# NVIDIA/nccl

Measured on AMD Instinct MI355X. Metric: all-reduce bus GB/s (device-resident), 256 MiB fp32, 1/2/4/8 MI355X, higher is better.
Workload: dtype f32; 1 GPU; ncclAllReduce sum fp32, 256 MiB, world_size=1 (the metric's size at N=1); collective=ncclAllReduce, op=sum, bytes_per_rank=268435456, count=67108864, n_ranks=1, out_of_place=True

## Files before the change

### nccl_amd/csrc/enqueue.cc

```cpp
#include <errno.h>
#include <stdio.h>
#include <stdlib.h>
#include <string.h>

#include <algorithm>
#include <cmath>

#include "core.h"

namespace ncclamd {

int typeSize(ncclDataType_t t) {
  switch (t) {
    case ncclInt8: case ncclUint8: case ncclFloat8e4m3: case ncclFloat8e5m2: return 1;
    case ncclFloat16: case ncclBfloat16: return 2;
    case ncclInt32: case ncclUint32: case ncclFloat32: return 4;
    case ncclInt64: case ncclUint64: case ncclFloat64: return 8;
    default: return -1;
  }
}

static uint16_t hostF32ToHalf(float f);
static uint16_t hostF32ToBf16(float f);
static uint8_t hostF32ToFp8(float f, bool e5m2);
// ... 258 lines not shown
      if (!strcmp(a, "*")) lo = 1, hi = NCCL_AMD_MAX_RANKS;
      else if (end != a && *end == '\0' && nr >= 1 && nr <= NCCL_AMD_MAX_RANKS) lo = hi = (int)nr;
      if (lo && okB && okC && okD) {
        for (int n = lo; n <= hi; n++) {
          if (vb >= 0) t->tableLL[n] = vb;
          if (vc >= 0) t->tableLL128[n] = vc;
          if (vd >= 0) t->tableOneShot[n] = vd;
        }
        rows++;
        continue;
      }
    }
    WARN("NCCL_AMD_SIZE_TABLE=%s:%d: expected 'nranks|* ll ll128 oneshot' (bytes, K/M/G, '-' = built-in); line ignored",
         path, lineNo);
    good = false;
  }
  fclose(f);
  INFO("NCCL_AMD_SIZE_TABLE=%s: %d rows applied", path, rows);
  return good;
}

int linkChannelBudget(int n) {
  if (n < 3) return 0;
  const double bLinkGBps = 76.8, wgGBps = 23.0, headroom = 2.0;
  const double need = (2.5 * n - 1.0) * bLinkGBps / wgGBps * headroom;
  int c = 32;
  while (c < need && c < NCCL_AMD_MAX_CHANNELS) c *= 2;
  return c;
}

int coResidentChannelCap(int minCUs, int ranksPerGpu) {
  if (minCUs < 1) minCUs = 256;
  if (ranksPerGpu < 1) ranksPerGpu = 1;
  const int cap = ranksPerGpu == 1 ? 2 * minCUs : minCUs / ranksPerGpu;
  return cap < 1 ? 1 : cap;
}

void resolveLinkChannels(CommTuning* t, int nranks, bool userMaxCTAs) {
  const int64_t env = paramInt("NCCL_AMD_LINK_CHANNELS", -1);
  t->linkChannels = env >= 0 ? (int)env : userMaxCTAs ? 0 : linkChannelBudget(nranks);
}

void resolveFence(CommTuning* t, bool oneDevice) {
  if (t->p2pFence < 0 && oneDevice) t->protoFlags |= 8;
}

static bool isHostMemory(const void* p) {
// ... 763 lines not shown
```

### nccl_amd/csrc/kernels.h

```cpp
#pragma once
#include <hip/hip_runtime.h>

#include <algorithm>
#include <type_traits>

#include "core.h"
#include "numerics.h"

namespace ncclamd {

typedef unsigned int u32x4 __attribute__((ext_vector_type(4)));
constexpr int kThreads = 512;
#define kCoResident __attribute__((amdgpu_waves_per_eu(4)))

extern bool gKernelLog;
void kernelLogNote(const void* fn, unsigned grid, unsigned block);
#define NCCL_AMD_LAUNCH(K, G, B, SH, ST, ...)                                                  \
  do {                                                                                          \
    if (::ncclamd::gKernelLog) ::ncclamd::kernelLogNote((const void*)(K), (G).x, (B).x);      \
    hipLaunchKernelGGL(K, G, B, SH, ST, __VA_ARGS__);                                           \
  } while (0)


__device__ __forceinline__ uint64_t clockTicks() { return __builtin_amdgcn_s_memrealtime(); }

__device__ __forceinline__ void storeRemote(void* p, u32x4 v) {
  asm volatile("global_store_dwordx4 %0, %1, off sc0 sc1\n\ts_nop 1" ::"v"(p), "v"(v) : "memory");
}
__device__ __forceinline__ void drainStores() { asm volatile("s_waitcnt vmcnt(0)" ::: "memory"); }

#ifndef NCCL_AMD_BUFFER_STORES
#define NCCL_AMD_BUFFER_STORES 1
#endif
constexpr int kSysWriteThrough = 1 | 16;
__device__ __forceinline__ __amdgpu_buffer_rsrc_t remoteRsrc(const void* base) {
  const uint64_t b = (uint64_t)base;
  const uint32_t lo = __builtin_amdgcn_readfirstlane((uint32_t)b);
  const uint32_t hi = __builtin_amdgcn_readfirstlane((uint32_t)(b >> 32));
  return __builtin_amdgcn_make_buffer_rsrc((void*)(((uint64_t)hi << 32) | lo), 0, -1, 0x00020000);
}
__device__ __forceinline__ void storeRemoteAt(__amdgpu_buffer_rsrc_t r, uint32_t byteOff, u32x4 v) {
  __builtin_amdgcn_raw_buffer_store_b128(v, r, byteOff, 0, kSysWriteThrough);
}

#ifndef NCCL_AMD_LOCAL_WT
#define NCCL_AMD_LOCAL_WT 0
#endif
struct LocalStore {
  __amdgpu_buffer_rsrc_t r;
  u32x4* d;
  __device__ __forceinline__ LocalStore(void* dst, uint64_t base) : d((u32x4*)dst + base) {
    if (NCCL_AMD_LOCAL_WT) r = remoteRsrc(d);
  }
  __device__ __forceinline__ void put(uint32_t k, u32x4 v) {
    if (NCCL_AMD_LOCAL_WT) __builtin_amdgcn_raw_buffer_store_b128(v, r, k * 16u, 0, kSysWriteThrough);
    else __builtin_nontemporal_store(v, d + k);
  }
};

template <typename T>
__device__ __forceinline__ void storeRemoteElt(T* p, T v) {
  if constexpr (sizeof(T) == 1) {
    uint32_t x = 0;
    __builtin_memcpy(&x, &v, 1);
    asm volatile("global_store_byte %0, %1, off sc0 sc1\n\ts_nop 1" ::"v"(p), "v"(x) : "memory");
  } else if constexpr (sizeof(T) == 2) {
    uint32_t x = 0;
    __builtin_memcpy(&x, &v, 2);
    asm volatile("global_store_short %0, %1, off sc0 sc1\n\ts_nop 1" ::"v"(p), "v"(x) : "memory");
  } else if constexpr (sizeof(T) == 4) {
    uint32_t x;
    __builtin_memcpy(&x, &v, 4);
    asm volatile("global_store_dword %0, %1, off sc0 sc1\n\ts_nop 1" ::"v"(p), "v"(x) : "memory");
  } else {
    uint64_t x;
    __builtin_memcpy(&x, &v, 8);
    asm volatile("global_store_dwordx2 %0, %1, off sc0 sc1\n\ts_nop 1" ::"v"(p), "v"(x) : "memory");
  }
}
// ... 101 lines not shown
#ifndef NCCL_AMD_COPY_UNROLL
#define NCCL_AMD_COPY_UNROLL 8
#endif
constexpr int kCopyUnroll = NCCL_AMD_COPY_UNROLL;
#ifndef NCCL_AMD_FOLD_UNROLL
#define NCCL_AMD_FOLD_UNROLL 4
#endif
constexpr int kFoldUnroll = NCCL_AMD_FOLD_UNROLL;
#ifndef NCCL_AMD_FOLD_UNROLL_SWAR
#define NCCL_AMD_FOLD_UNROLL_SWAR 2
#endif
#ifndef NCCL_AMD_FOLD_UNROLL_1B
#define NCCL_AMD_FOLD_UNROLL_1B 2
#endif
constexpr int kFoldUnrollSwar = NCCL_AMD_FOLD_UNROLL_SWAR;
constexpr int kFoldUnroll1B = NCCL_AMD_FOLD_UNROLL_1B;
#ifndef NCCL_AMD_FOLD_REPACK
#define NCCL_AMD_FOLD_REPACK 1
#endif
#ifndef NCCL_AMD_FOLD_PREFETCH
#define NCCL_AMD_FOLD_PREFETCH 1
#endif

template <typename T, bool REMOTE>
__device__ __forceinline__ void copyRange(void* dst, const void* src, uint64_t nbytes, bool aligned) {
  if (aligned) {
    uint64_t npk = nbytes >> 4;
    const u32x4* s = (const u32x4*)src;
    u32x4* d = (u32x4*)dst;
    constexpr int U = kCopyUnroll;
    uint64_t i = threadIdx.x;
    for (; i + (U - 1) * kThreads < npk; i += U * kThreads) {
      u32x4 v[U];
#pragma unroll
      for (int u = 0; u < U; u++) v[u] = __builtin_nontemporal_load(s + i + u * kThreads);
      LocalStore ls(dst, i - threadIdx.x);
      __amdgpu_buffer_rsrc_t rd;
      if (REMOTE && NCCL_AMD_BUFFER_STORES) rd = remoteRsrc(d + (i - threadIdx.x));
#pragma unroll
      for (int u = 0; u < U; u++) {
        if (REMOTE && NCCL_AMD_BUFFER_STORES) storeRemoteAt(rd, (uint32_t)((threadIdx.x + u * kThreads) * 16), v[u]);
        else if (REMOTE) storeRemote(d + i + u * kThreads, v[u]);
        else ls.put(threadIdx.x + u * kThreads, v[u]);
      }
    }
    for (; i < npk; i += kThreads) {
      u32x4 v = __builtin_nontemporal_load(s + i);
      if (REMOTE && NCCL_AMD_BUFFER_STORES) storeRemoteAt(remoteRsrc(d + (i - threadIdx.x)), threadIdx.x * 16u, v);
      else if (REMOTE) storeRemote(d + i, v);
      else __builtin_nontemporal_store(v, d + i);
    }
    uint64_t done = npk << 4;
    uint64_t tail = (nbytes - done) / sizeof(T);
    if (threadIdx.x < tail) {
      const T* st = (const T*)((const char*)src + done);
      T* dt = (T*)((char*)dst + done);
      if (REMOTE) storeRemoteElt(dt + threadIdx.x, st[threadIdx.x]);
      else dt[threadIdx.x] = st[threadIdx.x];
    }
  } else {
    uint64_t n = nbytes / sizeof(T);
    const T* s = (const T*)src;
    T* d = (T*)dst;
    for (uint64_t i = threadIdx.x; i < n; i += kThreads) {
      if (REMOTE) storeRemoteElt(d + i, s[i]);
      else d[i] = s[i];
    }
  }
}

template <typename T>
__device__ __forceinline__ void copyRangeMulti(char* dstLocal, char* const* dstPush, int nPush, const void* src,
                                               uint64_t nbytes, bool aligned) {
  if (nPush == 1 && !dstLocal) return copyRange<T, true>(dstPush[0], src, nbytes, aligned);
  if (nPush == 0) return dstLocal ? copyRange<T, false>(dstLocal, src, nbytes, aligned) : void();
  if (aligned) {
    const uint64_t npk = nbytes >> 4;
    const u32x4* s = (const u32x4*)src;
    constexpr int U = kCopyUnroll;
    uint64_t i = threadIdx.x;
    for (; i + (U - 1) * kThreads < npk; i += U * kThreads) {
      u32x4 v[U];
#pragma unroll
      for (int u = 0; u < U; u++) v[u] = __builtin_nontemporal_load(s + i + u * kThreads);
      if (dstLocal) {
        LocalStore ls(dstLocal, i - threadIdx.x);
#pragma unroll
        for (int u = 0; u < U; u++) ls.put(threadIdx.x + u * kThreads, v[u]);
      }
      for (int p = 0; p < nPush; p++) {
        u32x4* d = (u32x4*)dstPush[p];
        if (NCCL_AMD_BUFFER_STORES) {
          const __amdgpu_buffer_rsrc_t rd = remoteRsrc(d + (i - threadIdx.x));
#pragma unroll
          for (int u = 0; u < U; u++) storeRemoteAt(rd, (uint32_t)((threadIdx.x + u * kThreads) * 16), v[u]);
        } else {
#pragma unroll
          for (int u = 0; u < U; u++) storeRemote(d + i + u * kThreads, v[u]);
        }
      }
    }
    for (; i < npk; i += kThreads) {
      const u32x4 v = __builtin_nontemporal_load(s + i);
      if (dstLocal) __builtin_nontemporal_store(v, (u32x4*)dstLocal + i);
      for (int p = 0; p < nPush; p++) {
        u32x4* d = (u32x4*)dstPush[p];
        if (NCCL_AMD_BUFFER_STORES) storeRemoteAt(remoteRsrc(d + (i - threadIdx.x)), threadIdx.x * 16u, v);
        else storeRemote(d + i, v);
      }
    }
    const uint64_t done = npk << 4;
    const uint64_t tail = (nbytes - done) / sizeof(T);
    if (threadIdx.x < tail) {
      const T x = ((const T*)((const char*)src + done))[threadIdx.x];
      if (dstLocal) ((T*)(dstLocal + done))[threadIdx.x] = x;
      for (int p = 0; p < nPush; p++) storeRemoteElt((T*)(dstPush[p] + done) + threadIdx.x, x);
    }
  } else {
    const uint64_t n = nbytes / sizeof(T);
    const T* s = (const T*)src;
    for (uint64_t i = threadIdx.x; i < n; i += kThreads) {
      const T x = s[i];
      if (dstLocal) ((T*)dstLocal)[i] = x;
      for (int p = 0; p < nPush; p++) storeRemoteElt((T*)dstPush[p] + i, x);
    }
  }
}

template <typename T>
union PackU {
  u32x4 v;
  T e[16 / sizeof(T)];
};

template <typename T, int OP>
__device__ __forceinline__ u32x4 fp8PackF32(const Red<T, OP>& fn, int n, const char* const* src, uint64_t i) {
  constexpr bool E5 = IsFp8<T>::e5m2;
  u32x4 cur = __builtin_nontemporal_load((const u32x4*)src[0] + i), nxt = cur;
  float acc[16];
  for (int k = 0; k < n; k++) {
    if (k + 1 < n) nxt = __builtin_nontemporal_load((const u32x4*)src[k + 1] + i);
    float x[16];
#pragma unroll
    for (int w = 0; w < 4; w++) fp8Decode4<E5>(cur[w], x + 4 * w);
    if constexpr (OP == DEV_PREMULSUM) {
#pragma unroll
      for (int e = 0; e < 16; e += 2) {
        x[e] = opaqueF(x[e] * fn.s);
        x[e + 1] = opaqueF(x[e + 1] * fn.s);
        fp8RoundF<E5>(x[e], x[e + 1]);
      }
    }
    if (k == 0) {
#pragma unroll
      for (int e = 0; e < 16; e++) acc[e] = x[e];
    } else {
#pragma unroll
      for (int e = 0; e < 16; e += 2) {
        float r0, r1;
        if (OP == DEV_PROD) {
          r0 = opaqueF(x[e] * acc[e]);
          r1 = opaqueF(x[e + 1] * acc[e + 1]);
        } else if (OP == DEV_MINMAX) {
          r0 = fn.isMin ? minOrdered(x[e], acc[e]) : maxOrdered(x[e], acc[e]);
// ... 9 lines not shown
    }
    cur = nxt;
  }
  u32x4 out;
#pragma unroll
  for (int w = 0; w < 4; w++) out[w] = fp8Encode4<E5>(acc + 4 * w);
  return out;
}

#ifndef NCCL_AMD_FP8_H2
#define NCCL_AMD_FP8_H2 1
#endif
template <typename T, int OP>
__device__ __forceinline__ void foldFp8Packs(const Red<T, OP>& fn, int n, const char* const* src, uint64_t nelem,
                                             char* dstLocal, char* const* dstPush, int nPush) {
  constexpr bool E5 = IsFp8<T>::e5m2;
  const uint64_t npk = nelem / 16;
  const _Float16 sh = (_Float16)fn.s;
  const fp8h2 s2 = {sh, sh};
  const uint32_t scalarSpecial = (OP == DEV_PREMULSUM && !(__builtin_fabsf(fn.s) <= 65504.0f)) ? 1u : 0u;
  for (uint64_t i = threadIdx.x; i < npk; i += kThreads) {
    u32x4 out;
    if (NCCL_AMD_FP8_H2) {
      u32x4 cur = __builtin_nontemporal_load((const u32x4*)src[0] + i), nxt = cur;
      fp8h2 acc[8];
      uint32_t special = scalarSpecial;
      for (int k = 0; k < n; k++) {
        if (k + 1 < n) nxt = __builtin_nontemporal_load((const u32x4*)src[k + 1] + i);
        special |= fp8Special<E5>(cur[0]) | fp8Special<E5>(cur[1]) | fp8Special<E5>(cur[2]) | fp8Special<E5>(cur[3]);
        fp8h2 x[8];
#pragma unroll
        for (int w = 0; w < 4; w++) {
          x[2 * w] = fp8DecodeH2<E5>(cur[w], false);
          x[2 * w + 1] = fp8DecodeH2<E5>(cur[w], true);
        }
        if constexpr (OP == DEV_PREMULSUM) {
#pragma unroll
          for (int j = 0; j < 8; j++) x[j] = fp8RoundH2<E5>(x[j] * s2);
        }
        if (k == 0) {
#pragma unroll
          for (int j = 0; j < 8; j++) acc[j] = x[j];
        } else {
#pragma unroll
          for (int j = 0; j < 8; j++) {
            if (OP == DEV_MINMAX)
              acc[j] = fn.isMin ? __builtin_elementwise_minimum(x[j], acc[j]) : __builtin_elementwise_maximum(x[j], acc[j]);
            else if (OP == DEV_PROD)
              acc[j] = fp8RoundH2<E5>(x[j] * acc[j]);
            else
              acc[j] = fp8RoundH2<E5>(x[j] + acc[j]);
          }
        }
        cur = nxt;
      }
#pragma unroll
      for (int w = 0; w < 4; w++) out[w] = fp8EncodeH2x2<E5>(acc[2 * w], acc[2 * w + 1]);
      if (__builtin_expect(special != 0, 0)) out = fp8PackF32<T, OP>(fn, n, src, i);
    } else {
      out = fp8PackF32<T, OP>(fn, n, src, i);
    }
    if (dstLocal) __builtin_nontemporal_store(out, (u32x4*)dstLocal + i);
    for (int p = 0; p < nPush; p++) storeRemoteAt(remoteRsrc((u32x4*)dstPush[p] + (i - threadIdx.x)), threadIdx.x * 16u, out);
  }
  const uint64_t t = npk * 16 + threadIdx.x;
  if (t < nelem) {
    T a = fn.pre(((const T*)src[0])[t]);
    for (int k = 1; k < n; k++) a = fn.red(fn.pre(((const T*)src[k])[t]), a);
    a = fn.post(a);
    if (dstLocal) ((T*)dstLocal)[t] = a;
    for (int p = 0; p < nPush; p++) storeRemoteElt((T*)dstPush[p] + t, a);
  }
}

template <typename T, int OP, int UMAX = 64>
__device__ __forceinline__ void foldRange(const Red<T, OP>& fn, int n, const char* const* src, uint64_t nelem,
                                          char* dstLocal, char* const* dstPush, int nPush, bool aligned) {
  constexpr int EPP = 16 / sizeof(T);
  constexpr bool kSwarDiv = std::is_same<T, uint8_t>::value && OP == DEV_SUMPOSTDIV;
  constexpr bool kSwar = std::is_same<T, uint8_t>::value && (Swar8<OP>::ok || kSwarDiv);
  constexpr int kSwarOp = kSwarDiv ? DEV_SUM : OP;
  constexpr int U0 = sizeof(T) > 1 ? kFoldUnroll : kSwar ? kFoldUnrollSwar : kFoldUnroll1B;
  constexpr int U = U0 < UMAX ? U0 : UMAX;
  uint32_t swarMask = 0, divMagic = 0;
  if constexpr (kSwar && !kSwarDiv) swarMask = (uint32_t)(uint8_t)fn.arg * 0x01010101u;
  if constexpr (kSwarDiv) divMagic = swarDivMagic(fn.divisor);
  if constexpr (IsFp8<T>::value && NCCL_AMD_HW_FP8) {
    if (aligned) {
      foldFp8Packs<T, OP>(fn, n, src, nelem, dstLocal, dstPush, nPush);
      return;
    }
  }
  if (aligned) {
    const uint64_t npk = nelem / EPP;
    const uint64_t step = (uint64_t)U * kThreads;
    constexpr bool kPrefetch = NCCL_AMD_FOLD_PREFETCH && sizeof(T) > 1;
    PackU<T> acc[U], cur[U], nxt[U];
    if constexpr (kPrefetch) {
#pragma unroll
      for (int u = 0; u < U; u++) {
        uint64_t i = threadIdx.x + (uint64_t)u * kThreads;
        if (i < npk) cur[u].v = __builtin_nontemporal_load((const u32x4*)src[0] + i);
      }
    }
    for (uint64_t base = threadIdx.x; base < npk; base += step) {
      if constexpr (!kPrefetch) {
#pragma unroll
        for (int u = 0; u < U; u++) {
          uint64_t i = base + (uint64_t)u * kThreads;
          if (i < npk) cur[u].v = __builtin_nontemporal_load((const u32x4*)src[0] + i);
        }
      }
      for (int k = 0; k < n; k++) {
        const bool last = k + 1 == n;
        if (!last || (kPrefetch && base + step < npk)) {
          const u32x4* s = (const u32x4*)src[last ? 0 : k + 1];
          const uint64_t b = last ? base + step : base;
#pragma unroll
          for (int u = 0; u < U; u++) {
            uint64_t i = b + (uint64_t)u * kThreads;
            if (i < npk) nxt[u].v = __builtin_nontemporal_load(s + i);
          }
        }
#pragma unroll
        for (int u = 0; u < U; u++) {
          if constexpr (kSwar) {
#pragma unroll
            for (int w = 0; w < 4; w++) acc[u].v[w] = k == 0 ? cur[u].v[w] : Swar8<kSwarOp>::red(cur[u].v[w], acc[u].v[w], swarMask);
          } else {
#pragma unroll
            for (int e = 0; e < EPP; e++) {
              T x = fn.pre(cur[u].e[e]);
              acc[u].e[e] = k == 0 ? x : fn.red(x, acc[u].e[e]);
            }
            if constexpr (sizeof(T) == 1 && NCCL_AMD_FOLD_REPACK) asm volatile("" : "+v"(acc[u].v));
          }
          cur[u] = nxt[u];
        }
      }
      LocalStore ls(dstLocal, base - threadIdx.x);
#pragma unroll
      for (int u = 0; u < U; u++) {
        uint64_t i = base + (uint64_t)u * kThreads;
        if (i >= npk) continue;
        if constexpr (kSwarDiv) {
#pragma unroll
          for (int w = 0; w < 4; w++) acc[u].v[w] = swarDivBytes(acc[u].v[w], divMagic, fn.isSigned);
        } else {
#pragma unroll
          for (int e = 0; e < EPP; e++) acc[u].e[e] = fn.post(acc[u].e[e]);
        }
        if (dstLocal) ls.put(threadIdx.x + u * kThreads, acc[u].v);
        for (int p = 0; p < nPush; p++) {
          if (NCCL_AMD_BUFFER_STORES)
            storeRemoteAt(remoteRsrc((u32x4*)dstPush[p] + (base - threadIdx.x)), (threadIdx.x + u * kThreads) * 16u, acc[u].v);
          else storeRemote((u32x4*)dstPush[p] + i, acc[u].v);
        }
      }
    }
    const uint64_t t = npk * EPP + threadIdx.x;
    if (t < nelem) {
      T acc = fn.pre(((const T*)src[0])[t]);
      for (int k = 1; k < n; k++) acc = fn.red(fn.pre(((const T*)src[k])[t]), acc);
      acc = fn.post(acc);
      if (dstLocal) ((T*)dstLocal)[t] = acc;
      for (int p = 0; p < nPush; p++) storeRemoteElt((T*)dstPush[p] + t, acc);
    }
  } else {
    for (uint64_t t = threadIdx.x; t < nelem; t += kThreads) {
      T acc = fn.pre(((const T*)src[0])[t]);
      for (int k = 1; k < n; k++) acc = fn.red(fn.pre(((const T*)src[k])[t]), acc);
      acc = fn.post(acc);
      if (dstLocal) ((T*)dstLocal)[t] = acc;
      for (int p = 0; p < nPush; p++) storeRemoteElt((T*)dstPush[p] + t, acc);
// ... 183 lines not shown
            sh.pushPtr[np++] = dc.staging[p] + stagingOffset(dc, c, STG_AG, (int)(ctr(CTR_SEND_AG, p) % nSlots), me);
        }
      }
      sh.nPush = np;
      int first = (COLL == COLL_REDUCE ? a.root + 1 : me + 1) % n;
      for (int k = 0; k < n; k++) {
        int q = (first + k) % n;
        const int rslot = (int)(ctr(CTR_RECV_RS, q) % nSlots);
        sh.srcPtr[k] = q == me ? (const char*)a.sendbuff + myOff * ts
                     : rsPull  ? dc.staging[q] + stagingOffset(dc, c, STG_RS, rslot, me)
                               : dc.staging[me] + stagingOffset(dc, c, STG_RS, rslot, q);
      }
    }
    __syncthreads();
    if (COLL == COLL_AG) {
      const char* src = (const char*)a.sendbuff + lo * ts;
      char* dst = (char*)a.recvbuff + ((uint64_t)me * a.chunk + lo) * ts;
      copyRangeMulti<T>(dst != src ? dst : nullptr, sh.pushPtr, sh.nPush, src, nelem * ts, aligned);
    } else {
      char* dstLocal = nullptr;
      if (COLL == COLL_RS) dstLocal = (char*)a.recvbuff + lo * ts;
      else if (kAR || isRoot) dstLocal = (char*)a.recvbuff + myOff * ts;
      constexpr int kUMax = COLL != COLL_ARREF ? 64 : sizeof(T) == 1 ? 1 : sizeof(T) == 8 ? 2 : 64;
      foldRange<T, OP, kUMax>(fn, n, sh.srcPtr, nelem, dstLocal, sh.pushPtr, sh.nPush, aligned);
    }
    if (tid < NCCL_AMD_MAX_RANKS) {
      bool peer = tid < n && tid != me;
      bool dstPeer = peer && push && pushesTo(tid);
      sh.sigVal[tid] = dstPeer ? (agPull ? ctr(CTR_PULL_PUB, 0) : ctr(CTR_SEND_AG, tid)) + 1 : 0;
      sh.sigPtr[tid] = dstPeer ? dc.flags[tid] + flagIndex(c, agPull ? FLG_PULL_READY : FLG_AG_READY, me) : nullptr;
      bool ack = peer && COLL != COLL_AG;
      sh.sigVal[NCCL_AMD_MAX_RANKS + tid] = ack ? ctr(CTR_RECV_RS, tid) + 1 : 0;
      sh.sigPtr[NCCL_AMD_MAX_RANKS + tid] = ack ? dc.flags[tid] + flagIndex(c, FLG_RS_ACK, me) : nullptr;
    }
    __syncthreads();
    signalAll(sh.sigPtr, sh.sigVal, 2 * NCCL_AMD_MAX_RANKS, (push && !noRel) || forceRel);
    if (tid < n && tid != me) {
      if (COLL != COLL_AG) ctr(CTR_RECV_RS, tid)++;
      if (push && pushesTo(tid) && !agPull) ctr(CTR_SEND_AG, tid)++;
    }
    if (agPull && tid == 0) ctr(CTR_PULL_PUB, 0)++;
    __syncthreads();
    return true;
  }

  __device__ bool oneShotA(int step) {
    int tid = threadIdx.x;
// ... 26 lines not shown
    return true;
  }

  __device__ bool oneShotB(int step) {
    int tid = threadIdx.x;
    if (tid < NCCL_AMD_MAX_RANKS) sh.want[tid] = (tid < n && tid != me) ? ctr(CTR_RECV_RS, tid) + 1 : 0;
    __syncthreads();
    if (!waitAll<PROBE_STAGED>(dc, sh.st, myFlags(FLG_RS_READY), sh.want, !noAcq, &sh.probe)) return false;
    uint64_t lo, hi;
    sliceRange(a, cl, step, a.count, lo, hi);
    for (uint64_t x = lo; x < hi;) {
      const int owner = (int)(x / a.chunk);
      const uint64_t end = min(hi, (uint64_t)(owner + 1) * a.chunk);
      if (tid == 0) {
        int first = (owner + 1) % n;
        for (int k = 0; k < n; k++) {
          int q = (first + k) % n;
          sh.srcPtr[k] = q == me ? (const char*)a.sendbuff + x * ts
                                 : dc.staging[me] + stagingOffset(dc, c, STG_RS, (int)(ctr(CTR_RECV_RS, q) % nSlots), q) +
                                       (x - lo) * ts;
        }
      }
      __syncthreads();
      foldRange<T, OP>(fn, n, sh.srcPtr, end - x, (char*)a.recvbuff + x * ts, sh.pushPtr, 0, aligned);
      __syncthreads();
      x = end;
    }
    if (tid < NCCL_AMD_MAX_RANKS) {
      bool peer = tid < n && tid != me;
      sh.sigVal[tid] = peer ? ctr(CTR_RECV_RS, tid) + 1 : 0;
      sh.sigPtr[tid] = peer ? dc.flags[tid] + flagIndex(c, FLG_RS_ACK, me) : nullptr;
    }
    __syncthreads();
    signalAll(sh.sigPtr, sh.sigVal, NCCL_AMD_MAX_RANKS, forceRel);
    if (tid < n && tid != me) ctr(CTR_RECV_RS, tid)++;
    __syncthreads();
    return true;
  }

  __device__ bool phaseC(int step) {
    int tid = threadIdx.x;
    const int recvKind = agPull ? CTR_PULL_GOT : CTR_RECV_AG;
    if (tid < NCCL_AMD_MAX_RANKS) sh.want[tid] = (tid < n && tid != me) ? ctr(recvKind, tid) + 1 : 0;
    __syncthreads();
    if (!waitAll<PROBE_STAGED>(dc, sh.st, myFlags(agPull ? FLG_PULL_READY : FLG_AG_READY), sh.want, !noAcq, &sh.probe)) return false;
    for (int k = 1; k < n; k++) {
      const int q = peerAt(k);
// ... 1003 lines not shown
  if (a.regMode) {
    if (tid < n && tid != me) {
      sh.send[tid] = (const char*)loadFlag(dc.flags[me] + flagIndex(c, FLG_REG_SEND, tid));
      sh.recv[tid] = (char*)loadFlag(dc.flags[me] + flagIndex(c, FLG_REG_RECV, tid));
    }
    __syncthreads();
    if (tid == 0) {
      uintptr_t al = 0;
      for (int r = 0; r < n; r++) al |= (uintptr_t)sh.recv[r] | (COLL == SYM_AG ? 0 : (uintptr_t)sh.send[r]);
      sh.aligned = a.aligned != 0 && (al & 15) == 0;
    }
    __syncthreads();
    aligned = sh.aligned != 0;
  }
  if (ok && COLL == SYM_AR1) {
    uint64_t lo, hi;
    partOf(a.count, lo, hi);
    for (uint64_t x = lo; x < hi;) {
      const int owner = (int)(x / a.chunk);
      const uint64_t end = min(hi, (uint64_t)(owner + 1) * a.chunk);
      if (tid == 0)
        for (int k = 0; k < n; k++) sh.srcPtr[k] = sh.send[(owner + 1 + k) % n] + x * ts;
      __syncthreads();
      foldRange<T, OP>(fn, n, sh.srcPtr, end - x, sh.recv[me] + x * ts, nullptr, 0, aligned);
      __syncthreads();
      x = end;
    }
  } else if (ok && COLL != SYM_AG) {
    uint64_t lo, hi;
    partOf(blockLen(me), lo, hi);
    if (tid == 0)
      for (int k = 0; k < n; k++) sh.srcPtr[k] = sh.send[(me + 1 + k) % n] + ((uint64_t)me * a.chunk + lo) * ts;
    __syncthreads();
    char* dst = COLL == SYM_RS ? sh.recv[me] + lo * ts : sh.recv[me] + ((uint64_t)me * a.chunk + lo) * ts;
    const bool push = COLL == SYM_AR && wt;
    if (tid == 0) sh.pushPtr[0] = dst;
    __syncthreads();
    foldRange<T, OP>(fn, n, sh.srcPtr, hi - lo, push ? nullptr : dst, sh.pushPtr, push ? 1 : 0, aligned);
    __syncthreads();
  }
  if (ok && COLL == SYM_AR) {
    symSignal(dc, sh, c, FLG_SYM_MID, e, !wt || a.relFence);
    ok = symWait(dc, sh, c, FLG_SYM_MID, e, true);
  }
  if (ok && (COLL == SYM_AR || COLL == SYM_AG)) {
    for (int k = 1; k < n; k++) {
      const int q = chanPeer(me, n, c, k);
      uint64_t lo, hi;
      partOf(blockLen(q), lo, hi);
      const uint64_t off = ((uint64_t)q * a.chunk + lo) * ts;
      copyRange<T, false>(sh.recv[me] + off, sh.recv[q] + off, (hi - lo) * ts, aligned);
    }
    __syncthreads();
  }
  if (ok) {
    symSignal(dc, sh, c, FLG_SYM_DONE, e, false);
    ok = symWait(dc, sh, c, FLG_SYM_DONE, e, false);
  }
  (void)ok;
  if (tid == 0) dc.counters[ctrIndex(c, CTR_SYM, 0)] = e;
}
// ... 227 lines not shown
```

### nccl_amd/csrc/pipe.h

```cpp
#pragma once

namespace ncclamd {

enum PipeMode { MV_COPY = 0, MV_PRE = 1, MV_FOLD = 2, MV_FINAL = 3 };

__device__ bool waitWords(const DevComm& dc, ChanState& st, const uint64_t* const* ptr, const uint64_t* val, int n,
                          bool ACQ) {
  if (threadIdx.x < 64) {
    const int lane = threadIdx.x;
    const bool need = lane < n;
    uint64_t t0 = 0;
    uint32_t iter = 0;
    while (true) {
      bool ok = !need || loadFlag(ptr[lane]) >= val[lane];
      if (__all(ok)) break;
      if (iter == 0) t0 = clockTicks();
      __builtin_amdgcn_s_sleep(1);
      if ((++iter & 255) == 0) {
        bool bad = false;
        if (__hip_atomic_load(dc.abortFlag, __ATOMIC_RELAXED, __HIP_MEMORY_SCOPE_SYSTEM)) {
          if (lane == 0) reportError(dc, DERR_ABORT);
          bad = true;
        } else if (__hip_atomic_load(dc.errorWord, __ATOMIC_RELAXED, __HIP_MEMORY_SCOPE_SYSTEM)) {
          bad = true;
// ... 12 lines not shown
  }
  __syncthreads();
  return st.abort == 0;
}

template <typename T, int OP, int MODE>
__device__ __forceinline__ void pipeMove(const Red<T, OP>& fn, const char* acc, const char* x, uint64_t nelem,
                                         char* dstLocal, char* dstPush, bool aligned) {
  constexpr int EPP = 16 / sizeof(T);
  constexpr int U = sizeof(T) == 1 ? 1 : 4;
  auto elem = [&](T av, T xv) -> T {
    if (MODE == MV_COPY) return av;
    if (MODE == MV_PRE) return fn.pre(xv);
    T r = fn.red(fn.pre(xv), av);
    return MODE == MV_FINAL ? fn.post(r) : r;
  };
  uint64_t npk = aligned ? nelem / EPP : 0;
  for (uint64_t base = threadIdx.x; base < npk; base += (uint64_t)U * kThreads) {
    PackU<T> av[U], xv[U];
#pragma unroll
    for (int u = 0; u < U; u++) {
      const uint64_t i = base + (uint64_t)u * kThreads;
      if (i >= npk) continue;
      if (MODE != MV_PRE) av[u].v = __builtin_nontemporal_load((const u32x4*)acc + i);
      if (MODE != MV_COPY) xv[u].v = __builtin_nontemporal_load((const u32x4*)x + i);
    }
#pragma unroll
    for (int u = 0; u < U; u++) {
      const uint64_t i = base + (uint64_t)u * kThreads;
      if (i >= npk) continue;
      PackU<T> o;
      if (MODE == MV_COPY) o = av[u];
      else
#pragma unroll
        for (int e = 0; e < EPP; e++) o.e[e] = elem(av[u].e[e], xv[u].e[e]);
      if (dstLocal) __builtin_nontemporal_store(o.v, (u32x4*)dstLocal + i);
      if (dstPush) {
        if (NCCL_AMD_BUFFER_STORES) storeRemoteAt(remoteRsrc(dstPush), (uint32_t)(i * 16), o.v);
        else storeRemote((u32x4*)dstPush + i, o.v);
      }
    }
  }
  for (uint64_t t = npk * EPP + threadIdx.x; t < nelem; t += kThreads) {
    const T av = MODE == MV_PRE ? T{} : ((const T*)acc)[t];
    const T xv = MODE == MV_COPY ? T{} : ((const T*)x)[t];
    const T o = elem(av, xv);
    if (dstLocal) ((T*)dstLocal)[t] = o;
    if (dstPush) storeRemoteElt((T*)dstPush + t, o);
  }
}

struct PipeShared {
  ChanState st;
  const uint64_t* waitPtr[2];
  uint64_t waitVal[2];
  uint64_t* sigPtr[2];
  uint64_t sigVal[2];
  int nWait;
};
// ... 190 lines not shown
```

Measured before the change: 7294 GB/s.

## Rewrite copy and fold loops with buffer loads, software pipelining, and address-space hints

Replaces the copy paths with a templated copyPacks that uses wave-uniform buffer loads and stores and double-buffers batches, so the load of one batch overlaps the store of the previous one. It adds a rank-count-specialized foldBatchesN that pipelines loads across source ranks for full batches, and tags pointers as global address space so the compiler emits global rather than flat instructions. It also raises the per-workgroup bandwidth estimate in the link channel budget, which lowers the channel count chosen for three or more ranks. At world size 1 the all-reduce is essentially a local copy, so the new copy path is the part that matters; the change costs more template instantiations, code size and register pressure.

```diff
diff --git a/nccl_amd/csrc/enqueue.cc b/nccl_amd/csrc/enqueue.cc
--- a/nccl_amd/csrc/enqueue.cc
+++ b/nccl_amd/csrc/enqueue.cc
@@ -304,7 +304,7 @@
 
 int linkChannelBudget(int n) {
   if (n < 3) return 0;
-  const double bLinkGBps = 76.8, wgGBps = 23.0, headroom = 2.0;
+  const double bLinkGBps = 76.8, wgGBps = 25.0, headroom = 2.0;
   const double need = (2.5 * n - 1.0) * bLinkGBps / wgGBps * headroom;
   int c = 32;
   while (c < need && c < NCCL_AMD_MAX_CHANNELS) c *= 2;
diff --git a/nccl_amd/csrc/kernels.h b/nccl_amd/csrc/kernels.h
--- a/nccl_amd/csrc/kernels.h
+++ b/nccl_amd/csrc/kernels.h
@@ -46,15 +46,44 @@
 #ifndef NCCL_AMD_LOCAL_WT
 #define NCCL_AMD_LOCAL_WT 0
 #endif
+typedef __attribute__((address_space(1))) u32x4 GPack;
+__device__ __forceinline__ uint64_t uniformAddr(const void* p) {
+  const uint64_t b = (uint64_t)p;
+  const uint32_t lo = __builtin_amdgcn_readfirstlane((uint32_t)b);
+  const uint32_t hi = __builtin_amdgcn_readfirstlane((uint32_t)(b >> 32));
+  return ((uint64_t)hi << 32) | lo;
+}
+__device__ __forceinline__ const GPack* globalPacks(const void* p) { return (const GPack*)uniformAddr(p); }
+__device__ __forceinline__ u32x4 loadPack(const GPack* p) { return __builtin_nontemporal_load(p); }
+constexpr int kNonTemporal = 2;
+struct BatchLoad {
+  __amdgpu_buffer_rsrc_t r;
+  __device__ __forceinline__ BatchLoad(const GPack* first) : r(__builtin_amdgcn_make_buffer_rsrc((void*)(uint64_t)first, 0, -1, 0x00020000)) {}
+  __device__ __forceinline__ u32x4 get(uint32_t lane, int u) const {
+    return __builtin_amdgcn_raw_buffer_load_b128(r, lane * 16u, u * kThreads * 16, kNonTemporal);
+  }
+};
+
 struct LocalStore {
   __amdgpu_buffer_rsrc_t r;
-  u32x4* d;
-  __device__ __forceinline__ LocalStore(void* dst, uint64_t base) : d((u32x4*)dst + base) {
-    if (NCCL_AMD_LOCAL_WT) r = remoteRsrc(d);
+  GPack* d;
+  __device__ __forceinline__ LocalStore(void* dst, uint64_t base) : d((GPack*)uniformAddr((u32x4*)dst + base)) {
+    if (NCCL_AMD_LOCAL_WT) r = remoteRsrc((u32x4*)dst + base);
   }
   __device__ __forceinline__ void put(uint32_t k, u32x4 v) {
     if (NCCL_AMD_LOCAL_WT) __builtin_amdgcn_raw_buffer_store_b128(v, r, k * 16u, 0, kSysWriteThrough);
     else __builtin_nontemporal_store(v, d + k);
+  }
+};
+template <bool REMOTE>
+struct BatchStore {
+  uint64_t first;
+  __device__ __forceinline__ BatchStore(void* p) : first(uniformAddr(p)) {}
+  __device__ __forceinline__ void put(uint32_t lane, int u, u32x4 v) const {
+    constexpr int policy = (REMOTE || NCCL_AMD_LOCAL_WT) ? kSysWriteThrough : kNonTemporal;
+    const __amdgpu_buffer_rsrc_t r =
+        __builtin_amdgcn_make_buffer_rsrc((void*)(first + (uint64_t)u * kThreads * 16), 0, -1, 0x00020000);
+    __builtin_amdgcn_raw_buffer_store_b128(v, r, lane * 16u, 0, policy);
   }
 };
 
@@ -202,108 +231,133 @@
 #define NCCL_AMD_FOLD_PREFETCH 1
 #endif
 
-template <typename T, bool REMOTE>
-__device__ __forceinline__ void copyRange(void* dst, const void* src, uint64_t nbytes, bool aligned) {
+template <typename T, bool LOCAL, int NPUSH>
+__device__ __forceinline__ void copyPacks(char* dstLocal, char* push0, char* const* dstPush, int nPush,
+                                          const void* src, uint64_t nbytes, bool aligned) {
   if (aligned) {
-    uint64_t npk = nbytes >> 4;
-    const u32x4* s = (const u32x4*)src;
-    u32x4* d = (u32x4*)dst;
     constexpr int U = kCopyUnroll;
-    uint64_t i = threadIdx.x;
-    for (; i + (U - 1) * kThreads < npk; i += U * kThreads) {
-      u32x4 v[U];
-#pragma unroll
-      for (int u = 0; u < U; u++) v[u] = __builtin_nontemporal_load(s + i + u * kThreads);
-      LocalStore ls(dst, i - threadIdx.x);
-      __amdgpu_buffer_rsrc_t rd;
-      if (REMOTE && NCCL_AMD_BUFFER_STORES) rd = remoteRsrc(d + (i - threadIdx.x));
-#pragma unroll
-      for (int u = 0; u < U; u++) {
-        if (REMOTE && NCCL_AMD_BUFFER_STORES) storeRemoteAt(rd, (uint32_t)((threadIdx.x + u * kThreads) * 16), v[u]);
-        else if (REMOTE) storeRemote(d + i + u * kThreads, v[u]);
-        else ls.put(threadIdx.x + u * kThreads, v[u]);
-      }
-    }
-    for (; i < npk; i += kThreads) {
-      u32x4 v = __builtin_nontemporal_load(s + i);
-      if (REMOTE && NCCL_AMD_BUFFER_STORES) storeRemoteAt(remoteRsrc(d + (i - threadIdx.x)), threadIdx.x * 16u, v);
-      else if (REMOTE) storeRemote(d + i, v);
-      else __builtin_nontemporal_store(v, d + i);
-    }
-    uint64_t done = npk << 4;
-    uint64_t tail = (nbytes - done) / sizeof(T);
-    if (threadIdx.x < tail) {
-      const T* st = (const T*)((const char*)src + done);
-      T* dt = (T*)((char*)dst + done);
-      if (REMOTE) storeRemoteElt(dt + threadIdx.x, st[threadIdx.x]);
-      else dt[threadIdx.x] = st[threadIdx.x];
-    }
-  } else {
-    uint64_t n = nbytes / sizeof(T);
-    const T* s = (const T*)src;
-    T* d = (T*)dst;
-    for (uint64_t i = threadIdx.x; i < n; i += kThreads) {
-      if (REMOTE) storeRemoteElt(d + i, s[i]);
-      else d[i] = s[i];
-    }
-  }
-}
-
-template <typename T>
-__device__ __forceinline__ void copyRangeMulti(char* dstLocal, char* const* dstPush, int nPush, const void* src,
-                                               uint64_t nbytes, bool aligned) {
-  if (nPush == 1 && !dstLocal) return copyRange<T, true>(dstPush[0], src, nbytes, aligned);
-  if (nPush == 0) return dstLocal ? copyRange<T, false>(dstLocal, src, nbytes, aligned) : void();
-  if (aligned) {
+    constexpr uint32_t B = U * kThreads;
     const uint64_t npk = nbytes >> 4;
-    const u32x4* s = (const u32x4*)src;
-    constexpr int U = kCopyUnroll;
-    uint64_t i = threadIdx.x;
-    for (; i + (U - 1) * kThreads < npk; i += U * kThreads) {
-      u32x4 v[U];
-#pragma unroll
-      for (int u = 0; u < U; u++) v[u] = __builtin_nontemporal_load(s + i + u * kThreads);
-      if (dstLocal) {
-        LocalStore ls(dstLocal, i - threadIdx.x);
-#pragma unroll
-        for (int u = 0; u < U; u++) ls.put(threadIdx.x + u * kThreads, v[u]);
-      }
-      for (int p = 0; p < nPush; p++) {
-        u32x4* d = (u32x4*)dstPush[p];
-        if (NCCL_AMD_BUFFER_STORES) {
-          const __amdgpu_buffer_rsrc_t rd = remoteRsrc(d + (i - threadIdx.x));
-#pragma unroll
-          for (int u = 0; u < U; u++) storeRemoteAt(rd, (uint32_t)((threadIdx.x + u * kThreads) * 16), v[u]);
-        } else {
-#pragma unroll
-          for (int u = 0; u < U; u++) storeRemote(d + i + u * kThreads, v[u]);
-        }
-      }
-    }
-    for (; i < npk; i += kThreads) {
-      const u32x4 v = __builtin_nontemporal_load(s + i);
-      if (dstLocal) __builtin_nontemporal_store(v, (u32x4*)dstLocal + i);
-      for (int p = 0; p < nPush; p++) {
-        u32x4* d = (u32x4*)dstPush[p];
-        if (NCCL_AMD_BUFFER_STORES) storeRemoteAt(remoteRsrc(d + (i - threadIdx.x)), threadIdx.x * 16u, v);
-        else storeRemote(d + i, v);
+    const uint64_t nfull = npk / B;
+    const uint32_t t = threadIdx.x;
+    const GPack* const s = globalPacks(src);
+    char* const dl = LOCAL ? (char*)uniformAddr(dstLocal) : nullptr;
+    char* const dp = NPUSH == 1 ? (char*)uniformAddr(push0) : nullptr;
+    auto load = [&](u32x4(&v)[U], uint64_t b) {
+      const BatchLoad bl(s + b * B);
+#pragma unroll
+      for (int u = 0; u < U; u++) v[u] = bl.get(t, u);
+    };
+    auto store = [&](const u32x4(&v)[U], uint64_t b) {
+      const uint64_t off = b * B * 16;
+      if (LOCAL) {
+        BatchStore<false> bs(dl + off);
+#pragma unroll
+        for (int u = 0; u < U; u++) bs.put(t, u, v[u]);
+      }
+      if (NPUSH == 1) {
+        BatchStore<true> bs(dp + off);
+#pragma unroll
+        for (int u = 0; u < U; u++) bs.put(t, u, v[u]);
+      }
+      if (NPUSH < 0) {
+        for (int p = 0; p < nPush; p++) {
+          BatchStore<true> bs(dstPush[p] + off);
+#pragma unroll
+          for (int u = 0; u < U; u++) bs.put(t, u, v[u]);
+        }
+      }
+    };
+    u32x4 va[U], vb[U];
+    if (nfull >= 2) {
+      load(vb, 0);
+      load(va, 1);
+      store(vb, 0);
+      uint64_t b = 1;
+      for (; b + 2 < nfull; b += 2) {
+        load(vb, b + 1);
+        store(va, b);
+        load(va, b + 2);
+        store(vb, b + 1);
+      }
+      if (b + 1 < nfull) {
+        load(vb, b + 1);
+        store(va, b);
+        store(vb, b + 1);
+      } else {
+        store(va, b);
+      }
+    } else if (nfull == 1) {
+      load(va, 0);
+      store(va, 0);
+    }
+    const uint32_t rem = (uint32_t)(npk - nfull * B);
+    if (rem) {
+      const BatchLoad bl(s + nfull * B);
+      const uint64_t off = nfull * B * 16;
+#pragma unroll
+      for (int u = 0; u < U; u++)
+        if (t + u * kThreads < rem) va[u] = bl.get(t, u);
+      if (LOCAL) {
+        BatchStore<false> bs(dl + off);
+#pragma unroll
+        for (int u = 0; u < U; u++)
+          if (t + u * kThreads < rem) bs.put(t, u, va[u]);
+      }
+      if (NPUSH == 1) {
+        BatchStore<true> bs(dp + off);
+#pragma unroll
+        for (int u = 0; u < U; u++)
+          if (t + u * kThreads < rem) bs.put(t, u, va[u]);
+      }
+      if (NPUSH < 0) {
+        for (int p = 0; p < nPush; p++) {
+          BatchStore<true> bs(dstPush[p] + off);
+#pragma unroll
+          for (int u = 0; u < U; u++)
+            if (t + u * kThreads < rem) bs.put(t, u, va[u]);
+        }
       }
     }
     const uint64_t done = npk << 4;
     const uint64_t tail = (nbytes - done) / sizeof(T);
-    if (threadIdx.x < tail) {
-      const T x = ((const T*)((const char*)src + done))[threadIdx.x];
-      if (dstLocal) ((T*)(dstLocal + done))[threadIdx.x] = x;
-      for (int p = 0; p < nPush; p++) storeRemoteElt((T*)(dstPush[p] + done) + threadIdx.x, x);
+    if (t < tail) {
+      const T x = ((const T*)((const char*)src + done))[t];
+      if (LOCAL) ((T*)(dstLocal + done))[t] = x;
+      if (NPUSH == 1) storeRemoteElt((T*)(push0 + done) + t, x);
+      if (NPUSH < 0)
+        for (int p = 0; p < nPush; p++) storeRemoteElt((T*)(dstPush[p] + done) + t, x);
     }
   } else {
     const uint64_t n = nbytes / sizeof(T);
     const T* s = (const T*)src;
     for (uint64_t i = threadIdx.x; i < n; i += kThreads) {
       const T x = s[i];
-      if (dstLocal) ((T*)dstLocal)[i] = x;
-      for (int p = 0; p < nPush; p++) storeRemoteElt((T*)dstPush[p] + i, x);
-    }
+      if (LOCAL) ((T*)dstLocal)[i] = x;
+      if (NPUSH == 1) storeRemoteElt((T*)push0 + i, x);
+      if (NPUSH < 0)
+        for (int p = 0; p < nPush; p++) storeRemoteElt((T*)dstPush[p] + i, x);
+    }
+  }
+}
+
+template <typename T, bool REMOTE>
+__device__ __forceinline__ void copyRange(void* dst, const void* src, uint64_t nbytes, bool aligned) {
+  if (REMOTE) copyPacks<T, false, 1>(nullptr, (char*)dst, nullptr, 0, src, nbytes, aligned);
+  else copyPacks<T, true, 0>((char*)dst, nullptr, nullptr, 0, src, nbytes, aligned);
+}
+
+template <typename T>
+__device__ __forceinline__ void copyRangeMulti(char* dstLocal, char* const* dstPush, int nPush, const void* src,
+                                               uint64_t nbytes, bool aligned) {
+  if (nPush == 0) {
+    if (dstLocal) copyPacks<T, true, 0>(dstLocal, nullptr, nullptr, 0, src, nbytes, aligned);
+  } else if (nPush == 1) {
+    if (dstLocal) copyPacks<T, true, 1>(dstLocal, dstPush[0], nullptr, 0, src, nbytes, aligned);
+    else copyPacks<T, false, 1>(nullptr, dstPush[0], nullptr, 0, src, nbytes, aligned);
+  } else {
+    if (dstLocal) copyPacks<T, true, -1>(dstLocal, nullptr, dstPush, nPush, src, nbytes, aligned);
+    else copyPacks<T, false, -1>(nullptr, nullptr, dstPush, nPush, src, nbytes, aligned);
   }
 }
 
@@ -316,10 +370,10 @@
 template <typename T, int OP>
 __device__ __forceinline__ u32x4 fp8PackF32(const Red<T, OP>& fn, int n, const char* const* src, uint64_t i) {
   constexpr bool E5 = IsFp8<T>::e5m2;
-  u32x4 cur = __builtin_nontemporal_load((const u32x4*)src[0] + i), nxt = cur;
+  u32x4 cur = loadPack((const GPack*)src[0] + i), nxt = cur;
   float acc[16];
   for (int k = 0; k < n; k++) {
-    if (k + 1 < n) nxt = __builtin_nontemporal_load((const u32x4*)src[k + 1] + i);
+    if (k + 1 < n) nxt = loadPack((const GPack*)src[k + 1] + i);
     float x[16];
 #pragma unroll
     for (int w = 0; w < 4; w++) fp8Decode4<E5>(cur[w], x + 4 * w);
@@ -375,11 +429,11 @@
   for (uint64_t i = threadIdx.x; i < npk; i += kThreads) {
     u32x4 out;
     if (NCCL_AMD_FP8_H2) {
-      u32x4 cur = __builtin_nontemporal_load((const u32x4*)src[0] + i), nxt = cur;
+      u32x4 cur = loadPack((const GPack*)src[0] + i), nxt = cur;
       fp8h2 acc[8];
       uint32_t special = scalarSpecial;
       for (int k = 0; k < n; k++) {
-        if (k + 1 < n) nxt = __builtin_nontemporal_load((const u32x4*)src[k + 1] + i);
+        if (k + 1 < n) nxt = loadPack((const GPack*)src[k + 1] + i);
         special |= fp8Special<E5>(cur[0]) | fp8Special<E5>(cur[1]) | fp8Special<E5>(cur[2]) | fp8Special<E5>(cur[3]);
         fp8h2 x[8];
 #pragma unroll
@@ -413,7 +467,7 @@
     } else {
       out = fp8PackF32<T, OP>(fn, n, src, i);
     }
-    if (dstLocal) __builtin_nontemporal_store(out, (u32x4*)dstLocal + i);
+    if (dstLocal) __builtin_nontemporal_store(out, (GPack*)dstLocal + i);
     for (int p = 0; p < nPush; p++) storeRemoteAt(remoteRsrc((u32x4*)dstPush[p] + (i - threadIdx.x)), threadIdx.x * 16u, out);
   }
   const uint64_t t = npk * 16 + threadIdx.x;
@@ -426,18 +480,110 @@
   }
 }
 
-template <typename T, int OP, int UMAX = 64>
+template <typename T, int OP>
+struct FoldPack {
+  static constexpr int EPP = 16 / sizeof(T);
+  static constexpr bool kSwarDiv = std::is_same<T, uint8_t>::value && OP == DEV_SUMPOSTDIV;
+  static constexpr bool kSwar = std::is_same<T, uint8_t>::value && (Swar8<OP>::ok || kSwarDiv);
+  static constexpr int kSwarOp = kSwarDiv ? DEV_SUM : OP;
+  const Red<T, OP>& fn;
+  uint32_t swarMask = 0, divMagic = 0;
+  __device__ __forceinline__ FoldPack(const Red<T, OP>& f) : fn(f) {
+    if constexpr (kSwar && !kSwarDiv) swarMask = (uint32_t)(uint8_t)fn.arg * 0x01010101u;
+    if constexpr (kSwarDiv) divMagic = swarDivMagic(fn.divisor);
+  }
+  __device__ __forceinline__ void fold(PackU<T>& acc, const PackU<T>& cur, bool first) const {
+    if constexpr (kSwar) {
+#pragma unroll
+      for (int w = 0; w < 4; w++) acc.v[w] = first ? cur.v[w] : Swar8<kSwarOp>::red(cur.v[w], acc.v[w], swarMask);
+    } else {
+#pragma unroll
+      for (int e = 0; e < EPP; e++) {
+        T x = fn.pre(cur.e[e]);
+        acc.e[e] = first ? x : fn.red(x, acc.e[e]);
+      }
+      if constexpr (sizeof(T) == 1 && NCCL_AMD_FOLD_REPACK) asm volatile("" : "+v"(acc.v));
+    }
+  }
+  __device__ __forceinline__ void finish(PackU<T>& acc) const {
+    if constexpr (kSwarDiv) {
+#pragma unroll
+      for (int w = 0; w < 4; w++) acc.v[w] = swarDivBytes(acc.v[w], divMagic, fn.isSigned);
+    } else {
+#pragma unroll
+      for (int e = 0; e < EPP; e++) acc.e[e] = fn.post(acc.e[e]);
+    }
+  }
+};
+
+template <typename T, int OP, int U, bool LOCAL, bool PUSH, int N>
+__device__ __forceinline__ uint64_t foldBatchesN(const FoldPack<T, OP>& fp, const char* const* src, uint64_t npk,
+                                                 char* dstLocal, char* push0) {
+  constexpr uint32_t B = U * kThreads;
+  const uint64_t nfull = npk / B;
+  if (nfull == 0) return 0;
+  const uint32_t t = threadIdx.x;
+  const GPack* sp[N];
+#pragma unroll
+  for (int k = 0; k < N; k++) sp[k] = globalPacks(src[k]);
+  char* const dl = LOCAL ? (char*)uniformAddr(dstLocal) : nullptr;
+  char* const dp = PUSH ? (char*)uniformAddr(push0) : nullptr;
+  PackU<T> r[2][U], acc[U];
+  auto load = [&](PackU<T>(&v)[U], const GPack* s, uint64_t pk0) __attribute__((always_inline)) {
+    const BatchLoad bl(s + pk0);
+#pragma unroll
+    for (int u = 0; u < U; u++) v[u].v = bl.get(t, u);
+  };
+  auto batch = [&](uint64_t b) __attribute__((always_inline)) {
+    const uint64_t pk0 = b * B;
+    const uint64_t nextPk0 = b + 1 < nfull ? pk0 + B : pk0;
+#pragma unroll
+    for (int k = 0; k < N; k++) {
+      constexpr bool kEven = N % 2 == 0;
+      if (k + 1 < N) load(r[(k + 1) & 1], sp[(k + 1) % N], pk0);
+      else if (kEven) load(r[0], sp[0], nextPk0);
+#pragma unroll
+      for (int u = 0; u < U; u++) fp.fold(acc[u], r[k & 1][u], k == 0);
+      if (k + 1 == N && !kEven) load(r[0], sp[0], nextPk0);
+    }
+#pragma unroll
+    for (int u = 0; u < U; u++) fp.finish(acc[u]);
+    if (LOCAL) {
+      BatchStore<false> bs(dl + pk0 * 16);
+#pragma unroll
+      for (int u = 0; u < U; u++) bs.put(t, u, acc[u].v);
+    }
+    if (PUSH) {
+      BatchStore<true> bs(dp + pk0 * 16);
+#pragma unroll
+      for (int u = 0; u < U; u++) bs.put(t, u, acc[u].v);
+    }
+  };
+  constexpr bool kPeel = OP == DEV_SUM;
+  load(r[0], sp[0], 0);
+  if (kPeel) batch(0);
+  for (uint64_t b = kPeel ? 1 : 0; b < nfull; b++) batch(b);
+  return nfull * B;
+}
+template <typename T, int OP, int U, bool LOCAL, bool PUSH>
+__device__ __forceinline__ uint64_t foldBatches(const FoldPack<T, OP>& fp, int n, const char* const* src, uint64_t npk,
+                                                char* dstLocal, char* push0) {
+  switch (n) {
+    case 2: return foldBatchesN<T, OP, U, LOCAL, PUSH, 2>(fp, src, npk, dstLocal, push0);
+    case 4: return foldBatchesN<T, OP, U, LOCAL, PUSH, 4>(fp, src, npk, dstLocal, push0);
+    case 8: return foldBatchesN<T, OP, (U > 2 ? U / 2 : U), LOCAL, PUSH, 8>(fp, src, npk, dstLocal, push0);
+    default: return 0;
+  }
+}
+
+template <typename T, int OP, int UMAX = 64, int DSTS = 7>
 __device__ __forceinline__ void foldRange(const Red<T, OP>& fn, int n, const char* const* src, uint64_t nelem,
                                           char* dstLocal, char* const* dstPush, int nPush, bool aligned) {
   constexpr int EPP = 16 / sizeof(T);
-  constexpr bool kSwarDiv = std::is_same<T, uint8_t>::value && OP == DEV_SUMPOSTDIV;
-  constexpr bool kSwar = std::is_same<T, uint8_t>::value && (Swar8<OP>::ok || kSwarDiv);
-  constexpr int kSwarOp = kSwarDiv ? DEV_SUM : OP;
+  const FoldPack<T, OP> fp(fn);
+  constexpr bool kSwar = FoldPack<T, OP>::kSwar;
   constexpr int U0 = sizeof(T) > 1 ? kFoldUnroll : kSwar ? kFoldUnrollSwar : kFoldUnroll1B;
   constexpr int U = U0 < UMAX ? U0 : UMAX;
-  uint32_t swarMask = 0, divMagic = 0;
-  if constexpr (kSwar && !kSwarDiv) swarMask = (uint32_t)(uint8_t)fn.arg * 0x01010101u;
-  if constexpr (kSwarDiv) divMagic = swarDivMagic(fn.divisor);
   if constexpr (IsFp8<T>::value && NCCL_AMD_HW_FP8) {
     if (aligned) {
       foldFp8Packs<T, OP>(fn, n, src, nelem, dstLocal, dstPush, nPush);
@@ -447,47 +593,45 @@
   if (aligned) {
     const uint64_t npk = nelem / EPP;
     const uint64_t step = (uint64_t)U * kThreads;
+    uint64_t pk0 = 0;
+    if constexpr ((sizeof(T) > 1 || kSwar) && !(OP == DEV_MINMAX && Traits<T>::isFloat)) {
+      {
+        if ((DSTS & 4) && dstLocal && nPush == 1) pk0 = foldBatches<T, OP, U, true, true>(fp, n, src, npk, dstLocal, dstPush[0]);
+        else if ((DSTS & 1) && dstLocal && nPush == 0) pk0 = foldBatches<T, OP, U, true, false>(fp, n, src, npk, dstLocal, nullptr);
+        else if ((DSTS & 2) && !dstLocal && nPush == 1) pk0 = foldBatches<T, OP, U, false, true>(fp, n, src, npk, nullptr, dstPush[0]);
+      }
+    }
     constexpr bool kPrefetch = NCCL_AMD_FOLD_PREFETCH && sizeof(T) > 1;
     PackU<T> acc[U], cur[U], nxt[U];
     if constexpr (kPrefetch) {
 #pragma unroll
       for (int u = 0; u < U; u++) {
-        uint64_t i = threadIdx.x + (uint64_t)u * kThreads;
-        if (i < npk) cur[u].v = __builtin_nontemporal_load((const u32x4*)src[0] + i);
-      }
-    }
-    for (uint64_t base = threadIdx.x; base < npk; base += step) {
+        uint64_t i = pk0 + threadIdx.x + (uint64_t)u * kThreads;
+        if (i < npk) cur[u].v = loadPack((const GPack*)src[0] + i);
+      }
+    }
+    for (uint64_t base = pk0 + threadIdx.x; base < npk; base += step) {
       if constexpr (!kPrefetch) {
 #pragma unroll
         for (int u = 0; u < U; u++) {
           uint64_t i = base + (uint64_t)u * kThreads;
-          if (i < npk) cur[u].v = __builtin_nontemporal_load((const u32x4*)src[0] + i);
+          if (i < npk) cur[u].v = loadPack((const GPack*)src[0] + i);
         }
       }
       for (int k = 0; k < n; k++) {
         const bool last = k + 1 == n;
         if (!last || (kPrefetch && base + step < npk)) {
-          const u32x4* s = (const u32x4*)src[last ? 0 : k + 1];
+          const GPack* s = (const GPack*)src[last ? 0 : k + 1];
           const uint64_t b = last ? base + step : base;
 #pragma unroll
           for (int u = 0; u < U; u++) {
             uint64_t i = b + (uint64_t)u * kThreads;
-            if (i < npk) nxt[u].v = __builtin_nontemporal_load(s + i);
+            if (i < npk) nxt[u].v = loadPack(s + i);
           }
         }
 #pragma unroll
         for (int u = 0; u < U; u++) {
-          if constexpr (kSwar) {
-#pragma unroll
-            for (int w = 0; w < 4; w++) acc[u].v[w] = k == 0 ? cur[u].v[w] : Swar8<kSwarOp>::red(cur[u].v[w], acc[u].v[w], swarMask);
-          } else {
-#pragma unroll
-            for (int e = 0; e < EPP; e++) {
-              T x = fn.pre(cur[u].e[e]);
-              acc[u].e[e] = k == 0 ? x : fn.red(x, acc[u].e[e]);
-            }
-            if constexpr (sizeof(T) == 1 && NCCL_AMD_FOLD_REPACK) asm volatile("" : "+v"(acc[u].v));
-          }
+          fp.fold(acc[u], cur[u], k == 0);
           cur[u] = nxt[u];
         }
       }
@@ -496,13 +640,7 @@
       for (int u = 0; u < U; u++) {
         uint64_t i = base + (uint64_t)u * kThreads;
         if (i >= npk) continue;
-        if constexpr (kSwarDiv) {
-#pragma unroll
-          for (int w = 0; w < 4; w++) acc[u].v[w] = swarDivBytes(acc[u].v[w], divMagic, fn.isSigned);
-        } else {
-#pragma unroll
-          for (int e = 0; e < EPP; e++) acc[u].e[e] = fn.post(acc[u].e[e]);
-        }
+        fp.finish(acc[u]);
         if (dstLocal) ls.put(threadIdx.x + u * kThreads, acc[u].v);
         for (int p = 0; p < nPush; p++) {
           if (NCCL_AMD_BUFFER_STORES)
@@ -732,7 +870,8 @@
       if (COLL == COLL_RS) dstLocal = (char*)a.recvbuff + lo * ts;
       else if (kAR || isRoot) dstLocal = (char*)a.recvbuff + myOff * ts;
       constexpr int kUMax = COLL != COLL_ARREF ? 64 : sizeof(T) == 1 ? 1 : sizeof(T) == 8 ? 2 : 64;
-      foldRange<T, OP, kUMax>(fn, n, sh.srcPtr, nelem, dstLocal, sh.pushPtr, sh.nPush, aligned);
+      constexpr int kDsts = COLL == COLL_RS ? 1 : kAR ? 4 : 3;
+      foldRange<T, OP, kUMax, kDsts>(fn, n, sh.srcPtr, nelem, dstLocal, sh.pushPtr, sh.nPush, aligned);
     }
     if (tid < NCCL_AMD_MAX_RANKS) {
       bool peer = tid < n && tid != me;
@@ -805,7 +944,7 @@
         }
       }
       __syncthreads();
-      foldRange<T, OP>(fn, n, sh.srcPtr, end - x, (char*)a.recvbuff + x * ts, sh.pushPtr, 0, aligned);
+      foldRange<T, OP, 64, 1>(fn, n, sh.srcPtr, end - x, (char*)a.recvbuff + x * ts, sh.pushPtr, 0, aligned);
       __syncthreads();
       x = end;
     }
@@ -1855,7 +1994,7 @@
       if (tid == 0)
         for (int k = 0; k < n; k++) sh.srcPtr[k] = sh.send[(owner + 1 + k) % n] + x * ts;
       __syncthreads();
-      foldRange<T, OP>(fn, n, sh.srcPtr, end - x, sh.recv[me] + x * ts, nullptr, 0, aligned);
+      foldRange<T, OP, 64, 1>(fn, n, sh.srcPtr, end - x, sh.recv[me] + x * ts, nullptr, 0, aligned);
       __syncthreads();
       x = end;
     }
@@ -1869,7 +2008,7 @@
     const bool push = COLL == SYM_AR && wt;
     if (tid == 0) sh.pushPtr[0] = dst;
     __syncthreads();
-    foldRange<T, OP>(fn, n, sh.srcPtr, hi - lo, push ? nullptr : dst, sh.pushPtr, push ? 1 : 0, aligned);
+    foldRange<T, OP, 64, COLL == SYM_AR ? 3 : 1>(fn, n, sh.srcPtr, hi - lo, push ? nullptr : dst, sh.pushPtr, push ? 1 : 0, aligned);
     __syncthreads();
   }
   if (ok && COLL == SYM_AR) {
diff --git a/nccl_amd/csrc/pipe.h b/nccl_amd/csrc/pipe.h
--- a/nccl_amd/csrc/pipe.h
+++ b/nccl_amd/csrc/pipe.h
@@ -58,8 +58,8 @@
     for (int u = 0; u < U; u++) {
       const uint64_t i = base + (uint64_t)u * kThreads;
       if (i >= npk) continue;
-      if (MODE != MV_PRE) av[u].v = __builtin_nontemporal_load((const u32x4*)acc + i);
-      if (MODE != MV_COPY) xv[u].v = __builtin_nontemporal_load((const u32x4*)x + i);
+      if (MODE != MV_PRE) av[u].v = loadPack((const GPack*)acc + i);
+      if (MODE != MV_COPY) xv[u].v = loadPack((const GPack*)x + i);
     }
 #pragma unroll
     for (int u = 0; u < U; u++) {
@@ -70,7 +70,7 @@
       else
 #pragma unroll
         for (int e = 0; e < EPP; e++) o.e[e] = elem(av[u].e[e], xv[u].e[e]);
-      if (dstLocal) __builtin_nontemporal_store(o.v, (u32x4*)dstLocal + i);
+      if (dstLocal) __builtin_nontemporal_store(o.v, (GPack*)dstLocal + i);
       if (dstPush) {
         if (NCCL_AMD_BUFFER_STORES) storeRemoteAt(remoteRsrc(dstPush), (uint32_t)(i * 16), o.v);
         else storeRemote((u32x4*)dstPush + i, o.v);
```

Result: no change. 7291 GB/s (-0.0%).
